# KAISTChangmin/MPMAvatar

Hardware: AMD Instinct MI355X
Metric: MPM substeps/sec (500k particles, 256^3 grid) (higher is better)
Workload: dtype f32; 1 GPU; sheet-500k; scene_name=sheet-497762, n_particles=497762, n_elements=331298, n_vertices=166464, n_traditional=0, n_grid=256, mode=fast, parallelism=single, n_active_nodes=148974, n_collider_nodes=32541, n_mover_nodes=0, n_active_blocks=10021, rebins=10, fallback_particles=0

## Files before the change

mpmavatar_amd/csrc/fast_device.hpp:

```cpp
#pragma once
#include <hip/hip_ext.h>
#include <algorithm>
#include <array>
#include <cstring>
#include <string.h>
#include <cstdlib>
#include <dlfcn.h>

#include <rccl/rccl.h>

#include <atomic>
#include <thread>

#include <rocprim/device/device_radix_sort.hpp>
#include <rocprim/device/device_scan.hpp>

#include "bc.hpp"
#include "ctx.hpp"
#include "mpm_math.hpp"

namespace mpm {
inline namespace fk {


// ... 36 lines not shown
__device__ __forceinline__ void st3(const Soa &a, int c0, int i, V3 v) {
  a.at(c0, i) = v.x; a.at(c0 + 1, i) = v.y; a.at(c0 + 2, i) = v.z;
}
__device__ __forceinline__ M3 ld9(const Soa &a, int c0, int i) {
  return M3{a.at(c0, i), a.at(c0 + 1, i), a.at(c0 + 2, i), a.at(c0 + 3, i), a.at(c0 + 4, i),
            a.at(c0 + 5, i), a.at(c0 + 6, i), a.at(c0 + 7, i), a.at(c0 + 8, i)};
}
__device__ __forceinline__ void st9(const Soa &a, int c0, int i, const M3 &m) {
  a.at(c0, i) = m.a00; a.at(c0 + 1, i) = m.a01; a.at(c0 + 2, i) = m.a02; a.at(c0 + 3, i) = m.a10;
  a.at(c0 + 4, i) = m.a11; a.at(c0 + 5, i) = m.a12; a.at(c0 + 6, i) = m.a20; a.at(c0 + 7, i) = m.a21;
  a.at(c0 + 8, i) = m.a22;
}

enum { A_X = 0, A_V = 3, A_C = 6, A_MASS = 15, A_NC = 16 };
enum { N_STRESS = 0, N_VOL = 9, N_MU = 10, N_LAM = 11, N_NC = 12 };
enum { E_D = 0, E_RINV = 9, E_GAMMA = 12, E_KAPPA = 13, E_NC = 14 };
enum { T_F = 0, T_FT = 9, T_YS = 18, T_NC = 19 };
enum { GCH_MV = 4, GCH_VOUT = 4, GCH_COL = 8, GCH_MOV = 4 };

struct Bufs {
  Soa all, nv, el, tr;
  int *face_orig;
  int *sel;
};

struct Dims {
  int n_p, n_e, n_nv, n_v, n_t;
  int G, NB;
  float dx, inv_dx, grid_lim;
};
// ... 100 lines not shown

enum { SIG_PROGRESS = 1, SIG_DFLAG = 2, SIG_DSEQ = 3, SIG_RING0 = 8, SIG_RING_N = 16, SIG_WORDS = 32 };
static_assert(SIG_RING0 + SIG_RING_N <= SIG_WORDS && (SIG_RING_N & (SIG_RING_N - 1)) == 0, "signal ring must fit its buffer");
enum {
  CNT_FALLBACK = 0, CNT_DROPPED = 1,
  CNT_NCOL = 2, CNT_NMOV = 3,
  CNT_ACTIVE = 4,
  CNT_FACE = 5, CNT_DRIFT = 6,
  CNT_DRIFT_ALL = 7,
  CNT_EXP0 = 8, CNT_EXP1 = 9,
  CNT_LINK_TIMEOUT = 10, CNT_LINK_BAD = 11,
  CNT_LINK_VOTE = 12, CNT_LINK_VOTE_ALL = 13,
  CNT_BODY_MOVES = 14,
  CNT_PAR0 = 16,
  CNT_MMIN = 24, CNT_MMAX = 25, CNT_NSEL = 26,
  CNT_N = 32
};
constexpr int CNT_STATS_N = 8;
static_assert(CNT_NCOL + 1 == CNT_NMOV && CNT_LINK_TIMEOUT + 1 == CNT_LINK_BAD && CNT_LINK_VOTE + 1 == CNT_LINK_VOTE_ALL &&
              CNT_MMIN + 1 == CNT_MMAX && CNT_MMAX + 1 == CNT_NSEL, "counter slots that are copied or cleared as one range");
static_assert(CNT_ACTIVE < CNT_STATS_N && CNT_BODY_MOVES < CNT_PAR0 && CNT_PAR0 + 4 <= CNT_MMIN && CNT_NSEL < CNT_N, "counter layout");

constexpr int PEER_TAB = 8;
struct HaloIn {
  const int *slot;
  const float *buf[PEER_TAB];
  const int *sig[PEER_TAB];
  int n_peers, seq, ch;
};

struct GridPtrs {
  float *mv;
  float *vout;
  float *col;
  float *mov;
// ... 100 lines not shown
    if (m != 0.0f || px != 0.0f || py != 0.0f || pz != 0.0f) { pm[0] = 0.0f; pm[64] = 0.0f; pm[128] = 0.0f; pm[192] = 0.0f; }
    if (l == 0) z.m_flag[blk] = 0;
  }
  if (z.has_col && z.col_flag[blk]) {
    float *pc = z.col + ((size_t)blk * GCH_COL) * 64 + l;
    if (pc[0] != 0.0f) { pc[0] = 0.0f; pc[64] = 0.0f; pc[128] = 0.0f; pc[192] = 0.0f; pc[256] = 0.0f; pc[320] = 0.0f; pc[384] = 0.0f; }
    if (l == 0) z.col_flag[blk] = 0;
  }
  if (z.has_mov) {
    float *pv = z.mov + ((size_t)blk * GCH_MOV) * 64 + l;
    if (pv[0] != 0.0f) { pv[0] = 0.0f; pv[64] = 0.0f; pv[128] = 0.0f; pv[192] = 0.0f; }
  }
}


template <bool FINALIZE>
__device__ __forceinline__ void stress_elem_body(int e, const Bufs &b, F3 *ef, const Dims &d, float friction_coeff, const int *face_slot,
                                                 const SortKey *skeys, int blk_bits, int *counters, int step_id) {
  if (e >= d.n_e) return;
  const int sel = b.sel[e];
  int s1 = 0, s2 = 0, s3 = 0;
  SortKey sk = 0;
  M3 dm;
  if (FINALIZE) {
    s1 = face_slot[e]; s2 = face_slot[d.n_e + e]; s3 = face_slot[2 * d.n_e + e];
    sk = skeys[e];
    dm = m3_zero();
    dm.a02 = b.el.at(E_D + 2, e); dm.a12 = b.el.at(E_D + 5, e); dm.a22 = b.el.at(E_D + 8, e);
  } else {
    dm = ld9(b.el, E_D, e);
  }
  float gamma = b.el.at(E_GAMMA, e), kappa = b.el.at(E_KAPPA, e);
  V3 rinv = ld3(b.el, E_RINV, e);
  float vol = b.nv.at(N_VOL, e), mu = b.nv.at(N_MU, e), lam = b.nv.at(N_LAM, e);
  asm volatile("" : "+v"(s1), "+v"(s2), "+v"(s3), "+v"(sk), "+v"(dm.a02), "+v"(dm.a12), "+v"(dm.a22));
  asm volatile("" : "+v"(gamma), "+v"(kappa), "+v"(rinv.x), "+v"(rinv.y), "+v"(rinv.z), "+v"(vol), "+v"(mu), "+v"(lam));
  if (sel == 1) {
    for (int c = 0; c < 3; ++c) ef[c * d.n_e + e] = F3{0.0f, 0.0f, 0.0f};
    return;
  }
  V3 xe = v3(0, 0, 0), ve = v3(0, 0, 0);
  if (FINALIZE) {
    int v1 = d.n_nv + s1, v2 = d.n_nv + s2, v3i = d.n_nv + s3;
    V3 x1 = ld3(b.all, A_X, v1), x2 = ld3(b.all, A_X, v2), x3 = ld3(b.all, A_X, v3i);
    V3 u1 = ld3(b.all, A_V, v1), u2 = ld3(b.all, A_V, v2), u3 = ld3(b.all, A_V, v3i);
    ve = v3((u1.x + u2.x + u3.x) / 3.0f, (u1.y + u2.y + u3.y) / 3.0f, (u1.z + u2.z + u3.z) / 3.0f);
    xe = v3((x1.x + x2.x + x3.x) / 3.0f, (x1.y + x2.y + x3.y) / 3.0f, (x1.z + x2.z + x3.z) / 3.0f);
    V3 d1 = x2 - x1, d2 = x3 - x1;
    dm = m3_cols(d1, d2, v3(dm.a02, dm.a12, dm.a22));
  }
  QR3 q = qr_cloth(dm);
  float r02, r12, r22;
  V3 d3 = anisotropy_return_mapping(q, gamma, kappa, friction_coeff, r02, r12, r22);
  M3 stress;
  V3 f1, f2, f3;
  kirchhoff_anisotropy(q, r02, r12, r22, d3, rinv, vol, mu, lam, gamma, kappa, stress, f1, f2, f3);
  if (FINALIZE) {
    st3(b.all, A_V, e, ve);
    st3(b.all, A_X, e, xe);
  }
  b.el.at(E_D + 2, e) = d3.x; b.el.at(E_D + 5, e) = d3.y; b.el.at(E_D + 8, e) = d3.z;
  st9(b.nv, N_STRESS, e, stress);
  ef[e] = F3{f1.x, f1.y, f1.z};
  ef[d.n_e + e] = F3{f2.x, f2.y, f2.z};
  ef[2 * d.n_e + e] = F3{f3.x, f3.y, f3.z};
  if (FINALIZE) {
    int blk = key_block(sk, blk_bits);
    int oz = 4 * (blk % d.NB) - 1, oy = 4 * ((blk / d.NB) % d.NB) - 1, ox = 4 * (blk / (d.NB * d.NB)) - 1;
    int nbx = (int)(xe.x * d.inv_dx - 0.5f) - ox, nby = (int)(xe.y * d.inv_dx - 0.5f) - oy, nbz = (int)(xe.z * d.inv_dx - 0.5f) - oz;
    if (sel == 0 && ((unsigned)nbx > 5u || (unsigned)nby > 5u || (unsigned)nbz > 5u)) raise_drift(counters, step_id);
  }
}


constexpr int TS_I = 99, TS_J = 9;
constexpr int TILE_PAD = 768;
__device__ __forceinline__ int tile_idx(int i, int j, int k) { return i * TS_I + j * TS_J + k; }
// ... 139 lines not shown
```

mpmavatar_amd/csrc/fast_state.hpp:

```cpp
#pragma once
#include "g2p_device.hpp"

namespace mpm {


struct DistPeer : mpmhip_dist_peer {
  DistPeer() : mpmhip_dist_peer{} {}
  explicit DistPeer(const mpmhip_dist_peer &p) : mpmhip_dist_peer(p) {}
  float *link_local = nullptr, *link_remote = nullptr;
  int link_cap = 0;
  int *link_cnt = nullptr;
};

struct Rccl {
  void *h = nullptr;
  ncclResult_t (*GetUniqueId)(ncclUniqueId *) = nullptr;
  ncclResult_t (*CommInitRank)(ncclComm_t *, int, ncclUniqueId, int) = nullptr;
  ncclResult_t (*CommDestroy)(ncclComm_t) = nullptr;
  ncclResult_t (*GroupStart)() = nullptr;
  ncclResult_t (*GroupEnd)() = nullptr;
  ncclResult_t (*Send)(const void *, size_t, ncclDataType_t, int, ncclComm_t, hipStream_t) = nullptr;
  ncclResult_t (*Recv)(void *, size_t, ncclDataType_t, int, ncclComm_t, hipStream_t) = nullptr;
  ncclResult_t (*AllGather)(const void *, void *, size_t, ncclDataType_t, ncclComm_t, hipStream_t) = nullptr;
  ncclResult_t (*AllReduce)(const void *, void *, size_t, ncclDataType_t, ncclRedOp_t, ncclComm_t, hipStream_t) = nullptr;
// ... 43 lines not shown
    q.ghost_send = ghost_send; q.ghost_recv = ghost_recv;
    q.link_local = link_local; q.link_remote = link_remote; q.link_cap = link_cap; q.link_cnt = link_cnt;
    return q;
  }
};

constexpr int HALO_CHANNELS_MAX = 8;
inline int halo_channels(bool movers) { return movers ? 8 : 4; }
constexpr size_t halo_floats(size_t n_blocks, int channels) { return n_blocks * (size_t)channels * 64; }
constexpr size_t ghost_floats(size_t n_p, size_t n_e) { return 6 * n_p + 3 * n_e; }
constexpr int LINK_DATA0 = 32, LINK_FLAG_STRIDE = 16;
constexpr size_t link_arena_floats(int cap) { return (size_t)LINK_DATA0 + 2 * halo_floats((size_t)cap, HALO_CHANNELS_MAX); }
inline float *link_data(float *arena, int par, int cap) { return arena + LINK_DATA0 + (size_t)par * halo_floats((size_t)cap, HALO_CHANNELS_MAX); }
inline int *link_flag(float *arena, int par) { return (int *)arena + par * LINK_FLAG_STRIDE; }

constexpr int PIN_SCAN_N = 2, PIN_STATS_N = CNT_STATS_N, PIN_RCNT_N = RC_N, PIN_MASS_N = 3;
enum {
  PIN_SCAN = 0,
  PIN_STATS = PIN_SCAN + PIN_SCAN_N,
  PIN_ADJ_K = PIN_STATS + PIN_STATS_N,
  PIN_DIST_DRIFT,
  PIN_LINK_VOTE,
  PIN_LINK_TIMEOUT,
  PIN_HALO_MULTI,
  PIN_BODY_MOVES,
  PIN_RCNT,
  PIN_MASS = PIN_RCNT + PIN_RCNT_N,
  PIN_N = PIN_MASS + PIN_MASS_N
};
static_assert(PIN_SCAN + PIN_SCAN_N <= PIN_STATS && PIN_STATS + PIN_STATS_N <= PIN_ADJ_K && PIN_ADJ_K < PIN_DIST_DRIFT &&
              PIN_BODY_MOVES < PIN_RCNT && PIN_RCNT + PIN_RCNT_N <= PIN_MASS && PIN_MASS + PIN_MASS_N <= PIN_N,
// ... 128 lines not shown
      return true;
    }
    bool resize(size_t want) { if (!reserve(want)) return false; n = want; return true; }
    bool push_back(const T &v) { if (n == cap && !reserve(n + 1)) return false; p[n++] = v; return true; }
    void clear() { n = 0; }
    size_t size() const { return n; }
    T *data() { return p; }
    T &operator[](size_t i) { return p[i]; }
    T *begin() { return p; }
    T *end() { return p + n; }
    void release() { if (p) (void)hipHostFree(p); p = nullptr; n = cap = 0; }
  };
  Pinned<int> h_ranges, h_plist;
  Pinned<ChunkRec> h_chunks, h_chunks_g;
  bool elem_pending = false;
  bool all_simulated = false;
  int steps_since_rebin = 0;
  volatile int *h_sig = nullptr;
  unsigned sig_seq = 0;
  unsigned sig_at_rebin = 0;
  bool face_flag_seen = false;
  int host_lead = 6;
  bool have_order = false;
  int64_t rebins = 0;
  int rebin_interval = 32;
  bool adaptive_rebin = true;
  bool fuse_grid = true, fuse_trad = true;
  AccumRing acc;
  int64_t n_col_kept = 0;
  bool col_keep = true;
// ... 61 lines not shown
```

mpmavatar_amd/csrc/g2p_device.hpp:

```cpp
#pragma once
#include "p2g_device.hpp"

namespace mpm {
inline namespace fk {

struct G2PResult {
  V3 v;
  M3 C, F;
};

__device__ __forceinline__ G2PResult g2p_finish(const Stencil &s, const Dims &d, V3 nv, V3 Mx, V3 My, V3 Mz, V3 Fx, V3 Fy,
                                                V3 Fz) {
  G2PResult r;
  r.v = nv;
  float c4 = 4.0f * d.inv_dx;
  r.C = m3_cols(c4 * (Mx - s.fx.x * nv), c4 * (My - s.fx.y * nv), c4 * (Mz - s.fx.z * nv));
  r.F = m3_cols(d.inv_dx * Fx, d.inv_dx * Fy, d.inv_dx * Fz);
  return r;
}

#ifndef G2P_D3_SWEEP
#define G2P_D3_SWEEP 1
#endif
template <bool B128>
// ... 201 lines not shown
  WGT(g, 1, 0);
  __builtin_amdgcn_s_setprio(3);
  int w = xcd_slice(wg, n_chunks);
  if (w < 0) return;
  const ChunkRec cm = recs[w];
  asm volatile("" ::"s"(cm.e0), "s"(cm.t0), "s"(cm.v0));
  int blk = cm.blk, chunk = cm.chunk;
  int bz = blk % d.NB, by = (blk / d.NB) % d.NB, bx = blk / (d.NB * d.NB);
  int ox = 4 * bx - 1, oy = 4 * by - 1, oz = 4 * bz - 1;
  int cls = 0, s = 0;
  bool valid = cm.map(chunk * CHUNK + (int)threadIdx.x, cls, s);
  V3 x, d3;
  {
    int sx_ = valid ? s : 0, se = (valid && cls == 0) ? s : 0;
    x = ld3(b.all, A_X, sx_);
    d3 = v3(b.el.at(E_D + 2, se), b.el.at(E_D + 5, se), b.el.at(E_D + 8, se));
  }
  constexpr int NPT = TILE3 / PT;
  int nbk[NPT], nlk[NPT], hsl[NPT];
  float am[NPT], apx[NPT], apy[NPT], apz[NPT];
#pragma unroll
  for (int u = 0; u < NPT; ++u) {
    int t = (int)threadIdx.x + u * PT;
    int ti = t >> 6, tj = (t >> 3) & 7, tk = t & 7;
    int gx = ox + ti, gy = oy + tj, gz = oz + tk;
    bool in = in_grid(gx, gy, gz, d.G);
    nbk[u] = in ? blk_of(gx, gy, gz, d.NB) : -1;
    nlk[u] = loc_of(gx, gy, gz);
    am[u] = apx[u] = apy[u] = apz[u] = 0.0f;
    if (FUSED && !MFLAG) {
      const float *pm = g.mv + ((size_t)(in ? nbk[u] : blk) * GCH_MV) * 64 + nlk[u];
// ... 273 lines not shown
```

mpmavatar_amd/csrc/mpm_math.hpp:

```cpp
#pragma once
#include <hip/hip_runtime.h>

namespace mpm {

struct V3 {
  float x, y, z;
};
struct M3 {
  float a00, a01, a02, a10, a11, a12, a20, a21, a22;
};

__host__ __device__ __forceinline__ V3 v3(float x, float y, float z) { return V3{x, y, z}; }
__device__ __forceinline__ V3 operator+(V3 a, V3 b) { return V3{a.x + b.x, a.y + b.y, a.z + b.z}; }
__device__ __forceinline__ V3 operator-(V3 a, V3 b) { return V3{a.x - b.x, a.y - b.y, a.z - b.z}; }
__device__ __forceinline__ V3 operator*(float s, V3 a) { return V3{s * a.x, s * a.y, s * a.z}; }
__device__ __forceinline__ V3 operator*(V3 a, float s) { return V3{s * a.x, s * a.y, s * a.z}; }
__device__ __forceinline__ float dot(V3 a, V3 b) { return a.x * b.x + a.y * b.y + a.z * b.z; }
__device__ __forceinline__ V3 cross(V3 a, V3 b) {
  return V3{a.y * b.z - a.z * b.y, a.z * b.x - a.x * b.z, a.x * b.y - a.y * b.x};
}
__device__ __forceinline__ float length(V3 a) { return sqrtf(dot(a, a)); }
__device__ __forceinline__ V3 normalize(V3 a) {
  float l = length(a);
  float inv = l > 0.0f ? 1.0f / l : 0.0f;
// ... 283 lines not shown
    r22 = 1.0f;
  } else {
    float fn = kappa * (1.0f - q.r22) * (1.0f - q.r22);
    float ff = gamma * sqrtf(q.r02 * q.r02 + q.r12 * q.r12);
    if (ff > friction_coeff * fn) {
      r02 = q.r02 * friction_coeff * fn / ff;
      r12 = q.r12 * friction_coeff * fn / ff;
    }
  }
  float ax = r02 * q.q0.x, ay = r02 * q.q0.y, az = r02 * q.q0.z;
  float bx = r12 * q.q1.x, by = r12 * q.q1.y, bz = r12 * q.q1.z;
  float cx = r22 * q.q2.x, cy = r22 * q.q2.y, cz = r22 * q.q2.z;
  return v3((ax + bx) + cx, (ay + by) + cy, (az + bz) + cz);
}

__device__ __forceinline__ void kirchhoff_anisotropy(const QR3 &q, float r02, float r12, float r22, V3 d3, V3 Rinv,
                                                     float vol, float mu, float lam, float gamma, float kappa,
                                                     M3 &stress, V3 &f1, V3 &f2, V3 &f3) {
  float iD11 = Rinv.x, iD12 = Rinv.y, iD22 = Rinv.z;
  float F11 = q.r00 * iD11;
  float F12 = q.r00 * iD12 + q.r01 * iD22;
  float F22 = q.r11 * iD22;
  float hx = F11 + F22, hy = -F12;
  float hn = sqrtf(hx * hx + hy * hy);
  float c = hx / hn, s = hy / hn;
  float J = F11 * F22;
  float lj = lam * (J - 1.0f), m2 = 2.0f * mu;
  float K00 = m2 * (F11 - c) + lj * F22;
  float K01 = m2 * (F12 + s);
  float K11 = m2 * (F22 - c) + lj * F11;
  float dr13 = gamma * r02, dr23 = gamma * r12;
  float dr33 = (r22 > 1.0f) ? 0.0f : -kappa * (1.0f - r22) * (1.0f - r22);
  float k00 = K00 * F11 + K01 * F12 + dr13 * r02;
  float k01 = K01 * F22 + dr13 * r12;
  float k02 = dr13 * r22;
  float k11 = K11 * F22 + dr23 * r12;
  float k12 = dr23 * r22;
  float k22 = dr33 * r22;
  M3 K3s = M3{k00, k01, k02, k01, k11, k12, k02, k12, k22};
  float invdet = 1.0f / (F11 * F22 * r22);
  M3 Rinvm = invdet * M3{F22 * r22, 0.0f, 0.0f, -F12 * r22, F11 * r22, 0.0f, F12 * r12 - r02 * F22, -F11 * r12, F11 * F22};
  M3 Q = m3_cols(q.q0, q.q1, q.q2);
  M3 P = Q * K3s * Rinvm;
  V3 P1 = col0(P), P2 = col1(P), P3 = col2(P);
  f2 = (-vol) * (iD11 * P1 + iD12 * P2);
  f3 = (-vol * iD22) * P2;
  f1 = -1.0f * (f2 + f3);
  stress = vol * outer(P3, d3);
}

struct Stencil {
  int bx, by, bz;
  V3 fx;
  V3 w0, w1, w2;
  V3 dw0, dw1, dw2;
};

__device__ __forceinline__ Stencil make_stencil(V3 x, float inv_dx) {
  Stencil s;
  V3 g = inv_dx * x;
  s.bx = (int)(g.x - 0.5f);
  s.by = (int)(g.y - 0.5f);
  s.bz = (int)(g.z - 0.5f);
// ... 40 lines not shown
```

mpmavatar_amd/csrc/p2g.hip:

```cpp
#include "fast_state.hpp"

namespace mpm {

namespace {

template <bool FINALIZE>
__global__ void k_stress_elem(Bufs b, F3 *ef, Dims d, float friction_coeff, const int *face_slot,
                              const SortKey *skeys, int blk_bits, int *counters, int step_id) {
  stress_elem_body<FINALIZE>(blockIdx.x * blockDim.x + threadIdx.x, b, ef, d, friction_coeff, face_slot, skeys, blk_bits, counters, step_id);
}


__global__ void k_stress_trad(Bufs b, Dims d, mpmhip_model_scalars sc, float dt) {
  int t = blockIdx.x * blockDim.x + threadIdx.x;
  if (t >= d.n_t) return;
  int s = t + d.n_e;
  if (b.sel[s] != 0) return;
  M3 Ft = ld9(b.tr, T_FT, t), F, stress;
  float mu = b.nv.at(N_MU, s), lam = b.nv.at(N_LAM, s), ys = b.tr.at(T_YS, t);
  int m = sc.material;
  TradParams tp{m, sc.alpha, sc.hardening, sc.xi, sc.plastic_viscosity, sc.softening};
  traditional_update(Ft, tp, mu, lam, ys, dt, F, stress);
  if (m == 1 || m == 5) b.tr.at(T_YS, t) = ys;
  if (m == 5) { b.nv.at(N_MU, s) = mu; b.nv.at(N_LAM, s) = lam; }
  st9(b.tr, T_F, t, F);
  st9(b.nv, N_STRESS, s, stress);
}

__global__ __launch_bounds__(TPB) void k_stress_elem_splat(Bufs b, F3 *ef, Dims d, float friction_coeff, const int *face_slot,
                                                           const SortKey *skeys, int blk_bits, int n_splat, GridPtrs g, SplatArgs sa) {
  __shared__ double tile[4 * TILE_PAD];
  if ((int)blockIdx.x < n_splat) {
    col_splat_wg<1>(tile, sa, (int)blockIdx.x, d, g);
    return;
  }
  stress_elem_body<true>(((int)blockIdx.x - n_splat) * (int)blockDim.x + (int)threadIdx.x, b, ef, d, friction_coeff, face_slot, skeys,
                         blk_bits, g.counters, g.step_id);
}


template <int STEPS, bool TRAD, bool JT, bool FX>
__global__ __launch_bounds__(PT) void k_p2g(const ChunkRec *recs, int n_chunks, Bufs b, VAdj va, Dims d, float rpic, float dt,
                                             GridPtrs g, SplatArgs sa, TradParams tp) {
  __shared__ double tile[P2G_TILE_DOUBLES];
  __shared__ int esc[CHUNK];
  __shared__ int esc_n;
  __shared__ float red[8];
  p2g_body<STEPS, TRAD, JT, FX>(recs, n_chunks, b, va, d, rpic, dt, g, sa, tp, tile, esc, esc_n, red, (int)blockIdx.x);
}
}

void launch_p2g(mpmhip_ctx *c, bool trad, bool jt, unsigned grid, int n_chunks, float dt, const SplatArgs &sa, const TradParams &tp) {
// ... 4 lines not shown
#define P2G_ARGS grid, PT, f->chunks, n_chunks, b, f->va(), d, rpic, dt, f->g, sa, tp
  if (!f->p2g_fixed_now) {
    if (trad && jt) kstamp_launch(c, k_p2g<3, true, true, false>, P2G_ARGS);
    else if (trad) kstamp_launch(c, k_p2g<3, true, false, false>, P2G_ARGS);
    else kstamp_launch(c, k_p2g<3, false, false, false>, P2G_ARGS);
  } else if (trad && jt) kstamp_launch(c, k_p2g<P2G_STEPS, true, true, true>, P2G_ARGS);
  else if (trad) kstamp_launch(c, k_p2g<P2G_STEPS, true, false, true>, P2G_ARGS);
  else kstamp_launch(c, k_p2g<P2G_STEPS, false, false, true>, P2G_ARGS);
#undef P2G_ARGS
}
void launch_stress_elem(mpmhip_ctx *c, int mode, const SplatArgs &sa) {
  FastState *f = c->fast;
  const Dims &d = f->d;
  const Bufs &b = f->buf[f->cur];
  hipStream_t s = c->stream;
  if (mode == 2)
    kstamp_launch(c, k_stress_elem_splat, nblk(d.n_e) + (unsigned)sa.n_fbins, TPB, b, f->eforce, d, c->sc.friction_coeff, f->face_slot,
                  f->keys[1], f->blk_bits, sa.n_fbins, f->g, sa);
  else if (mode == 1)
    kstamp_launch(c, k_stress_elem<true>, nblk(d.n_e), TPB, b, f->eforce, d, c->sc.friction_coeff, f->face_slot, f->keys[1], f->blk_bits,
                  f->g.counters, f->g.step_id);
  else
    hipLaunchKernelGGL(k_stress_elem<false>, nblk(d.n_e), TPB, 0, s, b, f->eforce, d, c->sc.friction_coeff, f->face_slot, f->keys[1],
                       f->blk_bits, f->g.counters, f->g.step_id);
}
void launch_stress_trad(mpmhip_ctx *c, float dt) {
  FastState *f = c->fast;
  hipLaunchKernelGGL(k_stress_trad, nblk(f->d.n_t), TPB, 0, c->stream, f->buf[f->cur], f->d, c->sc, dt);
}

}
```

mpmavatar_amd/csrc/p2g_device.hpp:

```cpp
#pragma once
#include "fast_device.hpp"

namespace mpm {
inline namespace fk {

__device__ __forceinline__ bool splat_ok(int G, const Stencil &s) {
  return s.bx >= 0 && s.bx < G - 3 && s.by >= 0 && s.by < G - 3 && s.bz >= 0 && s.bz < G - 3;
}


__device__ __forceinline__ V3 face_centroid(const float *pts, const float *vel, float adv, const int32_t *idx, int f,
                                            V3 &p0, V3 &p1, V3 &p2) {
  int i0 = idx[3 * f], i1 = idx[3 * f + 1], i2 = idx[3 * f + 2];
  p0 = mesh_point(pts, vel, adv, i0); p1 = mesh_point(pts, vel, adv, i1); p2 = mesh_point(pts, vel, adv, i2);
  return v3((p0.x + p1.x + p2.x) / 3.0f, (p0.y + p1.y + p2.y) / 3.0f, (p0.z + p1.z + p2.z) / 3.0f);
}

struct FaceBin { int blk, start, cnt, pad; };

struct JointSplatArgs {
  const float *vel_t, *vel_v, *vel_f;
  int n_t, n_v, n_f;
  int off_t, off_v;
  const int *inv;
// ... 103 lines not shown
  int r;
  asm("v_cvt_rpi_i32_f32 %0, %1" : "=v"(r) : "v"(x));
  return r;
}

constexpr float DRIFT_LOOKAHEAD = 10.0f, DRIFT_LOOKAHEAD_DIST = 20.0f;
struct P2GRaw {
  V3 x, v;
  float mass, vol;
  M3 C, S;
  float mu, lam, ys;
  AdjBatch ab;
};
template <bool TRAD>
__device__ __forceinline__ P2GRaw p2g_issue(const Bufs &b, const VAdj &va, bool valid, int cls, int s, const Dims &d,
                                            bool w_nv, bool w_v) {
  P2GRaw r;
  int sa = valid ? s : 0;
  r.x = ld3(b.all, A_X, sa);
  r.mass = b.all.at(A_MASS, sa);
  r.C = ld9(b.all, A_C, sa);
  r.v = ld3(b.all, A_V, sa);
  r.S = m3_zero();
  r.vol = 1.0f;
  r.mu = r.lam = r.ys = 0.0f;
  if (w_nv) {
    int sn = (valid && cls != 2) ? s : 0;
    if (TRAD) {
      bool tr = valid && cls == 1;
      int t = tr ? s - d.n_e : 0;
      const float *base = tr ? b.tr.p + (size_t)T_FT * b.tr.n + t : b.nv.p + (size_t)N_STRESS * b.nv.n + sn;
      size_t st = tr ? (size_t)b.tr.n : (size_t)b.nv.n;
      r.S = M3{base[0], base[st], base[2 * st], base[3 * st], base[4 * st], base[5 * st], base[6 * st], base[7 * st], base[8 * st]};
      r.mu = b.nv.at(N_MU, sn);
      r.lam = b.nv.at(N_LAM, sn);
      if (d.n_t) r.ys = b.tr.at(T_YS, t);
    } else {
      r.S = ld9(b.nv, N_STRESS, sn);
    }
    r.vol = b.nv.at(N_VOL, sn);
  }
#pragma unroll
  for (int u = 0; u < ADJ_BATCH; ++u) r.ab.ent[u] = -1;
  if (w_v) r.ab = adj_load(va, (valid && cls == 2) ? s - d.n_nv : 0, 0);
  return r;
}
template <bool TRAD>
__device__ __forceinline__ P2GParticle p2g_finish(const P2GRaw &r, const Bufs &b, const VAdj &va, bool valid, int cls, int s,
                                                  const Dims &d, float rpic, float dt, bool w_v, const TradParams &tp) {
  V3 vf = v3(0, 0, 0);
  if (w_v) {
    vf = adj_gather(va, r.ab, vf);
    int vl = (valid && cls == 2) ? s - d.n_nv : 0;
    for (int k0 = ADJ_BATCH; k0 < va.K; k0 += ADJ_BATCH) vf = adj_gather(va, adj_load(va, vl, k0), vf);
  }
  P2GParticle q;
  q.s = make_stencil(r.x, d.inv_dx);
  q.mass = r.mass;
  q.mass_s = r.mass;
  M3 C = r.C;
  C = (1.0f - rpic) * C + (rpic / 2.0f) * (C - transpose(C));
  if (rpic < -0.001f) C = m3_zero();
  q.a0 = r.v - d.dx * (C * q.s.fx);
  q.Cdx = d.dx * C;
  q.Sdt = m3_zero();
  q.vfdt = v3(0, 0, 0);
  if (valid && cls == 0) {
    q.Sdt = (-dt * d.inv_dx) * r.S;
  } else if (valid && cls == 1) {
    M3 S = r.S;
    if (TRAD) {
      int t = s - d.n_e;
      M3 F;
      float mu = r.mu, lam = r.lam, ys = r.ys;
      traditional_update(r.S, tp, mu, lam, ys, dt, F, S);
      if (tp.material == 1 || tp.material == 5) b.tr.at(T_YS, t) = ys;
      if (tp.material == 5) { b.nv.at(N_MU, s) = mu; b.nv.at(N_LAM, s) = lam; }
      st9(b.tr, T_F, t, F);
      st9(b.nv, N_STRESS, s, S);
    }
    q.Sdt = (-dt * d.inv_dx * r.vol) * S;
  } else if (valid) {
    q.vfdt = dt * vf;
  }
  return q;
}
template <bool TRAD>
__device__ __forceinline__ P2GParticle p2g_load(const Bufs &b, const VAdj &va, int cls, int s, const Dims &d, float rpic,
                                                float dt, const TradParams &tp) {
  P2GRaw r = p2g_issue<TRAD>(b, va, true, cls, s, d, cls != 2, cls == 2);
  return p2g_finish<TRAD>(r, b, va, true, cls, s, d, rpic, dt, cls == 2, tp);
}

__device__ __forceinline__ int dpp_shr_i(int v, int old, int n) {
  switch (n) {
    case 1: return __builtin_amdgcn_update_dpp(old, v, 0x111, 0xf, 0xf, false);
    case 2: return __builtin_amdgcn_update_dpp(old, v, 0x112, 0xf, 0xf, false);
    case 4: return __builtin_amdgcn_update_dpp(old, v, 0x114, 0xf, 0xf, false);
    default: return __builtin_amdgcn_update_dpp(old, v, 0x118, 0xf, 0xf, false);
  }
}
__device__ __forceinline__ float dpp_shr_f(float v, int n) { return __int_as_float(dpp_shr_i(__float_as_int(v), 0, n)); }

struct SegMask {
  float m1, m2, m4, m8;
// ... 535 lines not shown
    WGT(g, 0, 6);
    return;
  }
  int w = xcd_slice(bid - (sa.e0 == 0 ? sa.n_extra : 0), n_chunks);
  if (w < 0) { wg_done(sa.pack); return; }
  if (g.stagger > 0 && bid < g.stagger_first) {
    int slot = (int)(__builtin_amdgcn_s_getreg(63492) & 0xfu) % g.stagger_groups;
    for (int i = 0; i < slot * g.stagger; ++i) __builtin_amdgcn_s_sleep(16);
  }
  const ChunkRec cm = recs[w];
  int blk = cm.blk, chunk = cm.chunk;
  int bz = blk % d.NB, by = (blk / d.NB) % d.NB, bx = blk / (d.NB * d.NB);
  int ox = 4 * bx - 1, oy = 4 * by - 1, oz = 4 * bz - 1;
  int cls = 0, s = 0;
  bool valid = cm.map(chunk * CHUNK + (int)threadIdx.x, cls, s);
  bool w_nv = __any(valid && cls != 2), w_v = __any(valid && cls == 2);
  if (DBG(g, 8)) w_v = false;
  if (DBG(g, 16)) w_nv = false;
  WGT(g, 0, 1);
  P2GRaw raw = p2g_issue<TRAD>(b, va, valid, cls, s, d, w_nv, w_v);
  for (int t = threadIdx.x; t < ((FX && !JT) ? 2 : 4) * TILE_PAD; t += PT) tile[t] = 0.0;
  if (threadIdx.x == 0) esc_n = 0;
  if (valid) {
    float la = g.lookahead * dt;
    int fx = (int)((raw.x.x + la * raw.v.x) * d.inv_dx - 0.5f) - ox, fy = (int)((raw.x.y + la * raw.v.y) * d.inv_dx - 0.5f) - oy,
        fz = (int)((raw.x.z + la * raw.v.z) * d.inv_dx - 0.5f) - oz;
    if ((unsigned)fx > 5u || (unsigned)fy > 5u || (unsigned)fz > 5u) raise_drift(g.counters, g.step_id);
  }
  WGT(g, 0, 2);
  P2GParticle q = p2g_finish<TRAD>(raw, b, va, valid, cls, s, d, rpic, dt, w_v, tp);
  FxScale fs{1.0f, 1.0f, 1.0f, 1.0f};
  if (FX) {
    float bm, bp;
    fx_bounds(q, valid, bm, bp);
    fs = fx_scales(bm, bp, red);
// ... 55 lines not shown
```

mpmavatar_amd/csrc/resort.hip:

```cpp
#include "fast_state.hpp"

namespace mpm {

namespace {


__global__ void k_import(mpmhip_state_ptrs st, mpmhip_model_ptrs md, Bufs b, const int *perm, Dims d, int dist) {
  int s = blockIdx.x * blockDim.x + threadIdx.x;
  if (s >= d.n_p) return;
  int o = perm[s];
  for (int c = 0; c < 3; ++c) b.all.at(A_X + c, s) = st.particle_x[3 * (size_t)o + c];
  for (int c = 0; c < 3; ++c) b.all.at(A_V + c, s) = st.particle_v[3 * (size_t)o + c];
  for (int c = 0; c < 9; ++c) b.all.at(A_C + c, s) = st.particle_C[9 * (size_t)o + c];
  b.all.at(A_MASS, s) = st.particle_mass[o];
  int sel = st.particle_selection[o];
  b.sel[s] = dist ? sel : (sel != 0 ? 1 : 0);
  if (s < d.n_nv) {
    for (int c = 0; c < 9; ++c) b.nv.at(N_STRESS + c, s) = st.particle_stress[9 * (size_t)o + c];
    b.nv.at(N_VOL, s) = st.particle_vol[o];
    b.nv.at(N_MU, s) = md.mu[o];
    b.nv.at(N_LAM, s) = md.lam[o];
    if (s < d.n_e) {
      for (int c = 0; c < 9; ++c) b.el.at(E_D + c, s) = st.particle_d[9 * (size_t)o + c];
      for (int c = 0; c < 3; ++c) b.el.at(E_RINV + c, s) = st.particle_R_inv[3 * (size_t)o + c];
      b.el.at(E_GAMMA, s) = md.gamma[o];
      b.el.at(E_KAPPA, s) = md.kappa[o];
      for (int c = 0; c < 3; ++c) b.face_orig[c * d.n_e + s] = (int)st.faces[3 * (size_t)o + c];
    } else {
      int t = s - d.n_e;
      for (int c = 0; c < 9; ++c) b.tr.at(T_F + c, t) = st.particle_F[9 * (size_t)o + c];
      for (int c = 0; c < 9; ++c) b.tr.at(T_FT + c, t) = st.particle_F_trial[9 * (size_t)o + c];
      b.tr.at(T_YS, t) = md.yield_stress[o];
    }
  }
}


__global__ void k_export(mpmhip_state_ptrs st, mpmhip_model_ptrs md, Bufs b, VAdj va, const int *perm,
                         Dims d, int export_model) {
  int s = blockIdx.x * blockDim.x + threadIdx.x;
  if (s >= d.n_p) return;
  int o = perm[s];
  for (int c = 0; c < 3; ++c) st.particle_x[3 * (size_t)o + c] = b.all.at(A_X + c, s);
  for (int c = 0; c < 3; ++c) st.particle_v[3 * (size_t)o + c] = b.all.at(A_V + c, s);
  for (int c = 0; c < 9; ++c) st.particle_C[9 * (size_t)o + c] = b.all.at(A_C + c, s);
  if (s < d.n_nv) {
    for (int c = 0; c < 9; ++c) st.particle_stress[9 * (size_t)o + c] = b.nv.at(N_STRESS + c, s);
    if (s < d.n_e) {
      for (int c = 0; c < 9; ++c) st.particle_d[9 * (size_t)o + c] = b.el.at(E_D + c, s);
    } else {
      int t = s - d.n_e;
      for (int c = 0; c < 9; ++c) st.particle_F[9 * (size_t)o + c] = b.tr.at(T_F + c, t);
      for (int c = 0; c < 9; ++c) st.particle_F_trial[9 * (size_t)o + c] = b.tr.at(T_FT + c, t);
      if (export_model) {
        md.yield_stress[o] = b.tr.at(T_YS, t);
        md.mu[o] = b.nv.at(N_MU, s);
        md.lam[o] = b.nv.at(N_LAM, s);
      }
    }
  } else {
    int v = s - d.n_nv;
    store_v3(st.vertex_force + 3 * (size_t)(o - d.n_nv), vertex_force(va, v));
// ... 235 lines not shown
}


__global__ void k_mass_span(const float *mass, const int *sel, int n, int *counters) {
  int i = blockIdx.x * blockDim.x + threadIdx.x;
  float m = (i < n && sel[i] == 0) ? mass[i] : 0.0f;
  int lo = m > 0.0f ? __float_as_int(m) : 0x7f7fffff, hi = m > 0.0f ? __float_as_int(m) : 0;
#pragma unroll
  for (int o = 32; o > 0; o >>= 1) { lo = min(lo, __shfl_xor(lo, o)); hi = max(hi, __shfl_xor(hi, o)); }
  if ((threadIdx.x & 63) == 0) { atomicMin(counters + CNT_MMIN, lo); atomicMax(counters + CNT_MMAX, hi); }
  unsigned long long ns = __ballot(i < n && sel[i] != 0);
  if ((threadIdx.x & 63) == 0 && ns) atomicAdd(counters + CNT_NSEL, (int)__popcll(ns));
}


__global__ __launch_bounds__(RS_TPB) void k_keys(Bufs b, Dims d, int kf, float lead, int ghost_g2p, SortKey *keys, int *iota, int *clear,
                                                 int n_clear, int *hist, int *gsum, int n_tiles, ZeroArgs z) {
  __shared__ int h[RS_BINS];
  if ((int)blockIdx.x >= n_tiles) {
    zero_blocks_wg(z, (int)blockIdx.x - n_tiles);
    return;
  }
  const int t = threadIdx.x, lane = t & 63, base = (int)blockIdx.x * RS_TILE;
  for (int i = (int)blockIdx.x * RS_TPB + t; i < n_clear; i += n_tiles * RS_TPB) clear[i] = 0;
  h[t] = 0;
  __syncthreads();
#pragma unroll
  for (int j = 0; j < RS_IPT; ++j) {
    int s = base + j * RS_TPB + t;
    bool in = s < d.n_p;
// ... 194 lines not shown
  return MPMHIP_OK;
}

int do_import(mpmhip_ctx *c) {
  FastState *f = c->fast;
  const Dims &d = f->d;
  if (!f->have_order) {
    if (d.n_p) hipLaunchKernelGGL(k_iota, nblk(d.n_p), TPB, 0, c->stream, f->perm[f->cur], d.n_p);
    f->have_order = true;
  }
  flush_g2p(c);
  if (d.n_p) {
    hipLaunchKernelGGL(k_import, nblk(d.n_p), TPB, 0, c->stream, c->st, c->md, f->buf[f->cur], f->perm[f->cur], d,
                       f->dist ? 1 : 0);
    MPM_HIP_CHECK(c, hipMemsetD32Async((hipDeviceptr_t)(f->g.counters + CNT_MMIN), 0x7f7fffff, 1, c->stream));
    MPM_HIP_CHECK(c, hipMemsetD32Async((hipDeviceptr_t)(f->g.counters + CNT_MMAX), 0, 2, c->stream));
    hipLaunchKernelGGL(k_mass_span, nblk(d.n_p), TPB, 0, c->stream, (const float *)c->st.particle_mass, (const int *)c->st.particle_selection,
                       d.n_p, f->g.counters);
    f->mass_span_pending = true;
  }
  if (d.n_e && d.n_v) {
    hipStream_t s = c->stream;
    MPM_HIP_CHECK(c, hipMemsetAsync(f->adj_cnt, 0, ((size_t)d.n_v + 1) * sizeof(int), s));
    hipLaunchKernelGGL(k_adj_build, nblk(d.n_e), TPB, 0, s, c->st.faces, d.n_e, d.n_v, f->adj_cnt, (int *)nullptr, 0, 0);
    hipLaunchKernelGGL(k_max_int, nblk(d.n_v), TPB, 0, s, f->adj_cnt, d.n_v, f->adj_cnt + d.n_v);
    MPM_HIP_CHECK(c, hipMemcpyAsync(f->h_pin + PIN_ADJ_K, f->adj_cnt + d.n_v, sizeof(int), hipMemcpyDeviceToHost, s));
    MPM_HIP_CHECK(c, hipStreamSynchronize(s));
    int K = std::max(f->h_pin[PIN_ADJ_K], 1);
    if (K > f->adj_cap) {
      int rc2;
      if ((rc2 = dalloc(c, &f->adj_o, (size_t)K * d.n_v, false))) return rc2;
      if ((rc2 = dalloc(c, &f->adj_s, (size_t)K * d.n_v, false))) return rc2;
      f->adj_cap = K;
    }
    f->adj_K = K;
    MPM_HIP_CHECK(c, hipMemsetAsync(f->adj_o, 0xff, (size_t)K * d.n_v * sizeof(int), s));
    MPM_HIP_CHECK(c, hipMemsetAsync(f->adj_cnt, 0, (size_t)d.n_v * sizeof(int), s));
    hipLaunchKernelGGL(k_adj_build, nblk(d.n_e), TPB, 0, s, c->st.faces, d.n_e, d.n_v, f->adj_cnt, f->adj_o, K, 1);
    MPM_HIP_CHECK(c, hipMemsetAsync(f->eforce, 0, ((size_t)3 * d.n_e + 1) * sizeof(F3), s));
  }
  f->elem_pending = false;
  c->caller_dirty = false;
  c->internal_dirty = false;
  f->steps_since_rebin = 1 << 30;
  return MPMHIP_OK;
}

constexpr int RS_MAX_N = 1 << 21;
static bool sort_custom(const FastState *f, int n) { return !f->sort_rocprim && n <= RS_MAX_N; }
static int sort_passes(int bits) { return (bits + RS_BITS - 1) / RS_BITS; }
static int sort_input(const FastState *f, int n, int bits) { return sort_custom(f, n) ? 1 - (sort_passes(bits) & 1) : 0; }
static int sort_reserve(mpmhip_ctx *c, int n) {
  FastState *f = c->fast;
  const int tiles = (n + RS_TILE - 1) / RS_TILE, groups = (tiles + RS_GROUP - 1) / RS_GROUP;
  if (tiles > f->rs_tiles) {
    int rc;
// ... 122 lines not shown
                       cap_A, f->rcnt, (int)RC_NA, 2, (int *)nullptr, 0);
    hipLaunchKernelGGL(k_build_chunks, 1, 1024, 0, s, f->plist, f->ranges, cap_P, f->rcnt, f->chunks, f->chunks + cap_ch, cap_ch, f->g.counters);
    if (with_faces)
      hipLaunchKernelGGL(k_fbin_compact, nblk(cap_A), TPB, 0, s, f->alist, f->rcnt, cap_A, f->fb_start, f->fb_cnt, f->fbins, cap_fb);
    MPM_HIP_CHECK(c, hipMemcpyAsync(f->h_pin + PIN_RCNT, f->rcnt, PIN_RCNT_N * sizeof(int), hipMemcpyDeviceToHost, s));
    if (f->mass_span_pending)
      MPM_HIP_CHECK(c, hipMemcpyAsync(f->h_pin + PIN_MASS, f->g.counters + CNT_MMIN, PIN_MASS_N * sizeof(int), hipMemcpyDeviceToHost, s));
    MPM_HIP_CHECK(c, hipStreamSynchronize(s));
    if (f->mass_span_pending) {
      float lo, hi;
      const int *hm = f->h_pin + PIN_MASS;
      memcpy(&lo, hm, 4); memcpy(&hi, hm + (CNT_MMAX - CNT_MMIN), 4);
      f->mass_span = (hi > 0.0f && lo < 3.0e38f) ? hi / lo : 1.0f;
      f->p2g_fixed_now = f->p2g_fixed && (f->p2g_fixed_forced || std::max(f->mass_span, f->global_mass_span) <= 1.0e5f);
      f->all_simulated = hm[CNT_NSEL - CNT_MMIN] == 0;
      f->mass_span_pending = false;
    }
    const int *h = f->h_pin + PIN_RCNT;
    if (h[RC_OVER]) {
      f->cap_P = std::max(f->cap_P, std::min(nb, std::max(h[RC_NP], (h[RC_NCH] - d.n_p / CHUNK)) * 2 + 1024));
      if (h[RC_OVER] & ~1) f->cap_P = std::min(nb, f->cap_P * 2);
      continue;
    }
    f->n_P = h[RC_NP];
    f->n_A = h[RC_NA];
    f->acc.end_relist(relist, f->alist, f->n_A);
    f->n_chunks = h[RC_NCH];
    const bool any_ghost = h[RC_GHOST] != 0;
    f->n_chunks_g = any_ghost ? h[RC_NCHG] : f->n_chunks;
    f->chunks_g = any_ghost ? f->chunks + cap_ch : f->chunks;
// ... 15 lines not shown
  }
  f->sig_at_rebin = f->sig_seq;
  f->g.ab_flag = f->ab_flag;
  f->steps_since_rebin = 0;
  f->rebins += 1;
  return MPMHIP_OK;
}

int fast_pull(mpmhip_ctx *c) {
  FastState *f = c->fast;
  const Dims &d = f->d;
  flush_elements(c);
  if (d.n_p && f->have_order) {
    int m = c->sc.material;
    hipLaunchKernelGGL(k_export, nblk(d.n_p), TPB, 0, c->stream, c->st, c->md, f->buf[f->cur], f->va(),
                       f->perm[f->cur], d, (m == 1 || m == 5) ? 1 : 0);
  }
  c->internal_dirty = false;
  return MPMHIP_OK;
}
int fast_debug_sort(mpmhip_ctx *c, const uint32_t *keys_in, int n, int bits, uint32_t *keys_out, int32_t *order_out) {
  FastState *f = c->fast;
  if (n == 0) return MPMHIP_OK;
  unsigned *kb[2] = {nullptr, nullptr};
  int *vtmp = nullptr;
  auto done = [&](int rc) {
    for (void *p : {(void *)kb[0], (void *)kb[1], (void *)vtmp}) if (p) (void)hipFree(p);
    return rc;
  };
  MPM_HIP_CHECK(c, hipMalloc(&kb[0], (size_t)n * sizeof(unsigned)));
  if (hipMalloc(&kb[1], (size_t)n * sizeof(unsigned)) != hipSuccess || hipMalloc(&vtmp, (size_t)n * sizeof(int)) != hipSuccess)
// ... 14 lines not shown
```

Measured before the change: 16190 substeps/s.

## Store element stress as rank-one factors and hoist uniform material constants

```diff
diff --git a/mpmavatar_amd/csrc/fast_device.hpp b/mpmavatar_amd/csrc/fast_device.hpp
--- a/mpmavatar_amd/csrc/fast_device.hpp
+++ b/mpmavatar_amd/csrc/fast_device.hpp
@@ -74,6 +74,7 @@
 
 enum { A_X = 0, A_V = 3, A_C = 6, A_MASS = 15, A_NC = 16 };
 enum { N_STRESS = 0, N_VOL = 9, N_MU = 10, N_LAM = 11, N_NC = 12 };
+enum { N_P3 = N_STRESS, N_D3 = N_STRESS + 3 };
 enum { E_D = 0, E_RINV = 9, E_GAMMA = 12, E_KAPPA = 13, E_NC = 14 };
 enum { T_F = 0, T_FT = 9, T_YS = 18, T_NC = 19 };
 enum { GCH_MV = 4, GCH_VOUT = 4, GCH_COL = 8, GCH_MOV = 4 };
@@ -204,11 +205,13 @@
   CNT_BODY_MOVES = 14,
   CNT_PAR0 = 16,
   CNT_MMIN = 24, CNT_MMAX = 25, CNT_NSEL = 26,
+  CNT_EC_DIFF = 27, CNT_EC_VAL = 28,
   CNT_N = 32
 };
 constexpr int CNT_STATS_N = 8;
 static_assert(CNT_NCOL + 1 == CNT_NMOV && CNT_LINK_TIMEOUT + 1 == CNT_LINK_BAD && CNT_LINK_VOTE + 1 == CNT_LINK_VOTE_ALL &&
-              CNT_MMIN + 1 == CNT_MMAX && CNT_MMAX + 1 == CNT_NSEL, "counter slots that are copied or cleared as one range");
+              CNT_MMIN + 1 == CNT_MMAX && CNT_MMAX + 1 == CNT_NSEL && CNT_NSEL + 1 == CNT_EC_DIFF && CNT_EC_DIFF + 1 == CNT_EC_VAL &&
+              CNT_EC_VAL + 4 == CNT_N, "counter slots that are copied or cleared as one range");
 static_assert(CNT_ACTIVE < CNT_STATS_N && CNT_BODY_MOVES < CNT_PAR0 && CNT_PAR0 + 4 <= CNT_MMIN && CNT_NSEL < CNT_N, "counter layout");
 
 constexpr int PEER_TAB = 8;
@@ -339,9 +342,13 @@
 }
 
 
+struct ElemConsts {
+  float gamma, kappa, mu, lam;
+  int uniform;
+};
 template <bool FINALIZE>
 __device__ __forceinline__ void stress_elem_body(int e, const Bufs &b, F3 *ef, const Dims &d, float friction_coeff, const int *face_slot,
-                                                 const SortKey *skeys, int blk_bits, int *counters, int step_id) {
+                                                 const SortKey *skeys, int blk_bits, int *counters, int step_id, const ElemConsts &ec) {
   if (e >= d.n_e) return;
   const int sel = b.sel[e];
   int s1 = 0, s2 = 0, s3 = 0;
@@ -355,9 +362,13 @@
   } else {
     dm = ld9(b.el, E_D, e);
   }
-  float gamma = b.el.at(E_GAMMA, e), kappa = b.el.at(E_KAPPA, e);
   V3 rinv = ld3(b.el, E_RINV, e);
-  float vol = b.nv.at(N_VOL, e), mu = b.nv.at(N_MU, e), lam = b.nv.at(N_LAM, e);
+  float vol = b.nv.at(N_VOL, e);
+  float gamma = ec.gamma, kappa = ec.kappa, mu = ec.mu, lam = ec.lam;
+  if (!ec.uniform) {
+    gamma = b.el.at(E_GAMMA, e); kappa = b.el.at(E_KAPPA, e);
+    mu = b.nv.at(N_MU, e); lam = b.nv.at(N_LAM, e);
+  }
   asm volatile("" : "+v"(s1), "+v"(s2), "+v"(s3), "+v"(sk), "+v"(dm.a02), "+v"(dm.a12), "+v"(dm.a22));
   asm volatile("" : "+v"(gamma), "+v"(kappa), "+v"(rinv.x), "+v"(rinv.y), "+v"(rinv.z), "+v"(vol), "+v"(mu), "+v"(lam));
   if (sel == 1) {
@@ -377,15 +388,14 @@
   QR3 q = qr_cloth(dm);
   float r02, r12, r22;
   V3 d3 = anisotropy_return_mapping(q, gamma, kappa, friction_coeff, r02, r12, r22);
-  M3 stress;
   V3 f1, f2, f3;
-  kirchhoff_anisotropy(q, r02, r12, r22, d3, rinv, vol, mu, lam, gamma, kappa, stress, f1, f2, f3);
+  V3 P3 = kirchhoff_anisotropy_factor(q, r02, r12, r22, rinv, vol, mu, lam, gamma, kappa, f1, f2, f3);
   if (FINALIZE) {
     st3(b.all, A_V, e, ve);
     st3(b.all, A_X, e, xe);
   }
-  b.el.at(E_D + 2, e) = d3.x; b.el.at(E_D + 5, e) = d3.y; b.el.at(E_D + 8, e) = d3.z;
-  st9(b.nv, N_STRESS, e, stress);
+  st3(b.nv, N_P3, e, P3);
+  st3(b.nv, N_D3, e, d3);
   ef[e] = F3{f1.x, f1.y, f1.z};
   ef[d.n_e + e] = F3{f2.x, f2.y, f2.z};
   ef[2 * d.n_e + e] = F3{f3.x, f3.y, f3.z};
diff --git a/mpmavatar_amd/csrc/fast_state.hpp b/mpmavatar_amd/csrc/fast_state.hpp
--- a/mpmavatar_amd/csrc/fast_state.hpp
+++ b/mpmavatar_amd/csrc/fast_state.hpp
@@ -81,7 +81,7 @@
 inline float *link_data(float *arena, int par, int cap) { return arena + LINK_DATA0 + (size_t)par * halo_floats((size_t)cap, HALO_CHANNELS_MAX); }
 inline int *link_flag(float *arena, int par) { return (int *)arena + par * LINK_FLAG_STRIDE; }
 
-constexpr int PIN_SCAN_N = 2, PIN_STATS_N = CNT_STATS_N, PIN_RCNT_N = RC_N, PIN_MASS_N = 3;
+constexpr int PIN_SCAN_N = 2, PIN_STATS_N = CNT_STATS_N, PIN_RCNT_N = RC_N, PIN_MASS_N = CNT_N - CNT_MMIN;
 enum {
   PIN_SCAN = 0,
   PIN_STATS = PIN_SCAN + PIN_SCAN_N,
@@ -240,6 +240,8 @@
   Pinned<int> h_ranges, h_plist;
   Pinned<ChunkRec> h_chunks, h_chunks_g;
   bool elem_pending = false;
+  bool elem_stress_factored = false;
+  ElemConsts elem_consts{0.0f, 0.0f, 0.0f, 0.0f, 0};
   bool all_simulated = false;
   int steps_since_rebin = 0;
   volatile int *h_sig = nullptr;
diff --git a/mpmavatar_amd/csrc/g2p_device.hpp b/mpmavatar_amd/csrc/g2p_device.hpp
--- a/mpmavatar_amd/csrc/g2p_device.hpp
+++ b/mpmavatar_amd/csrc/g2p_device.hpp
@@ -239,7 +239,7 @@
   {
     int sx_ = valid ? s : 0, se = (valid && cls == 0) ? s : 0;
     x = ld3(b.all, A_X, sx_);
-    d3 = v3(b.el.at(E_D + 2, se), b.el.at(E_D + 5, se), b.el.at(E_D + 8, se));
+    d3 = ld3(b.nv, N_D3, se);
   }
   constexpr int NPT = TILE3 / PT;
   int nbk[NPT], nlk[NPT], hsl[NPT];
diff --git a/mpmavatar_amd/csrc/mpm_math.hpp b/mpmavatar_amd/csrc/mpm_math.hpp
--- a/mpmavatar_amd/csrc/mpm_math.hpp
+++ b/mpmavatar_amd/csrc/mpm_math.hpp
@@ -321,9 +321,11 @@
   return v3((ax + bx) + cx, (ay + by) + cy, (az + bz) + cz);
 }
 
-__device__ __forceinline__ void kirchhoff_anisotropy(const QR3 &q, float r02, float r12, float r22, V3 d3, V3 Rinv,
-                                                     float vol, float mu, float lam, float gamma, float kappa,
-                                                     M3 &stress, V3 &f1, V3 &f2, V3 &f3) {
+__device__ __forceinline__ M3 stress_from_factors(float vol, V3 P3, V3 d3) { return vol * outer(P3, d3); }
+
+__device__ __forceinline__ V3 kirchhoff_anisotropy_factor(const QR3 &q, float r02, float r12, float r22, V3 Rinv,
+                                                          float vol, float mu, float lam, float gamma, float kappa,
+                                                          V3 &f1, V3 &f2, V3 &f3) {
   float iD11 = Rinv.x, iD12 = Rinv.y, iD22 = Rinv.z;
   float F11 = q.r00 * iD11;
   float F12 = q.r00 * iD12 + q.r01 * iD22;
@@ -353,7 +355,13 @@
   f2 = (-vol) * (iD11 * P1 + iD12 * P2);
   f3 = (-vol * iD22) * P2;
   f1 = -1.0f * (f2 + f3);
-  stress = vol * outer(P3, d3);
+  return P3;
+}
+__device__ __forceinline__ void kirchhoff_anisotropy(const QR3 &q, float r02, float r12, float r22, V3 d3, V3 Rinv,
+                                                     float vol, float mu, float lam, float gamma, float kappa,
+                                                     M3 &stress, V3 &f1, V3 &f2, V3 &f3) {
+  V3 P3 = kirchhoff_anisotropy_factor(q, r02, r12, r22, Rinv, vol, mu, lam, gamma, kappa, f1, f2, f3);
+  stress = stress_from_factors(vol, P3, d3);
 }
 
 struct Stencil {
diff --git a/mpmavatar_amd/csrc/p2g.hip b/mpmavatar_amd/csrc/p2g.hip
--- a/mpmavatar_amd/csrc/p2g.hip
+++ b/mpmavatar_amd/csrc/p2g.hip
@@ -6,8 +6,8 @@
 
 template <bool FINALIZE>
 __global__ void k_stress_elem(Bufs b, F3 *ef, Dims d, float friction_coeff, const int *face_slot,
-                              const SortKey *skeys, int blk_bits, int *counters, int step_id) {
-  stress_elem_body<FINALIZE>(blockIdx.x * blockDim.x + threadIdx.x, b, ef, d, friction_coeff, face_slot, skeys, blk_bits, counters, step_id);
+                              const SortKey *skeys, int blk_bits, int *counters, int step_id, ElemConsts ec) {
+  stress_elem_body<FINALIZE>(blockIdx.x * blockDim.x + threadIdx.x, b, ef, d, friction_coeff, face_slot, skeys, blk_bits, counters, step_id, ec);
 }
 
 
@@ -28,14 +28,15 @@
 }
 
 __global__ __launch_bounds__(TPB) void k_stress_elem_splat(Bufs b, F3 *ef, Dims d, float friction_coeff, const int *face_slot,
-                                                           const SortKey *skeys, int blk_bits, int n_splat, GridPtrs g, SplatArgs sa) {
+                                                           const SortKey *skeys, int blk_bits, int n_splat, GridPtrs g, SplatArgs sa,
+                                                           ElemConsts ec) {
   __shared__ double tile[4 * TILE_PAD];
   if ((int)blockIdx.x < n_splat) {
     col_splat_wg<1>(tile, sa, (int)blockIdx.x, d, g);
     return;
   }
   stress_elem_body<true>(((int)blockIdx.x - n_splat) * (int)blockDim.x + (int)threadIdx.x, b, ef, d, friction_coeff, face_slot, skeys,
-                         blk_bits, g.counters, g.step_id);
+                         blk_bits, g.counters, g.step_id, ec);
 }
 
 
@@ -70,15 +71,17 @@
   const Dims &d = f->d;
   const Bufs &b = f->buf[f->cur];
   hipStream_t s = c->stream;
+  const ElemConsts &ec = f->elem_consts;
+  f->elem_stress_factored = true;
   if (mode == 2)
     kstamp_launch(c, k_stress_elem_splat, nblk(d.n_e) + (unsigned)sa.n_fbins, TPB, b, f->eforce, d, c->sc.friction_coeff, f->face_slot,
-                  f->keys[1], f->blk_bits, sa.n_fbins, f->g, sa);
+                  f->keys[1], f->blk_bits, sa.n_fbins, f->g, sa, ec);
   else if (mode == 1)
     kstamp_launch(c, k_stress_elem<true>, nblk(d.n_e), TPB, b, f->eforce, d, c->sc.friction_coeff, f->face_slot, f->keys[1], f->blk_bits,
-                  f->g.counters, f->g.step_id);
+                  f->g.counters, f->g.step_id, ec);
   else
     hipLaunchKernelGGL(k_stress_elem<false>, nblk(d.n_e), TPB, 0, s, b, f->eforce, d, c->sc.friction_coeff, f->face_slot, f->keys[1],
-                       f->blk_bits, f->g.counters, f->g.step_id);
+                       f->blk_bits, f->g.counters, f->g.step_id, ec);
 }
 void launch_stress_trad(mpmhip_ctx *c, float dt) {
   FastState *f = c->fast;
diff --git a/mpmavatar_amd/csrc/p2g_device.hpp b/mpmavatar_amd/csrc/p2g_device.hpp
--- a/mpmavatar_amd/csrc/p2g_device.hpp
+++ b/mpmavatar_amd/csrc/p2g_device.hpp
@@ -141,7 +141,7 @@
 };
 template <bool TRAD>
 __device__ __forceinline__ P2GRaw p2g_issue(const Bufs &b, const VAdj &va, bool valid, int cls, int s, const Dims &d,
-                                            bool w_nv, bool w_v) {
+                                            bool w_nv, bool w_v, bool w_t) {
   P2GRaw r;
   int sa = valid ? s : 0;
   r.x = ld3(b.all, A_X, sa);
@@ -158,12 +158,15 @@
       int t = tr ? s - d.n_e : 0;
       const float *base = tr ? b.tr.p + (size_t)T_FT * b.tr.n + t : b.nv.p + (size_t)N_STRESS * b.nv.n + sn;
       size_t st = tr ? (size_t)b.tr.n : (size_t)b.nv.n;
-      r.S = M3{base[0], base[st], base[2 * st], base[3 * st], base[4 * st], base[5 * st], base[6 * st], base[7 * st], base[8 * st]};
+      r.S = M3{base[0], base[st], base[2 * st], base[3 * st], base[4 * st], base[5 * st], 0.0f, 0.0f, 0.0f};
+      if (w_t) { r.S.a20 = base[6 * st]; r.S.a21 = base[7 * st]; r.S.a22 = base[8 * st]; }
       r.mu = b.nv.at(N_MU, sn);
       r.lam = b.nv.at(N_LAM, sn);
       if (d.n_t) r.ys = b.tr.at(T_YS, t);
     } else {
-      r.S = ld9(b.nv, N_STRESS, sn);
+      V3 s0 = ld3(b.nv, N_STRESS, sn), s1 = ld3(b.nv, N_STRESS + 3, sn), s2 = v3(0, 0, 0);
+      if (w_t) s2 = ld3(b.nv, N_STRESS + 6, sn);
+      r.S = M3{s0.x, s0.y, s0.z, s1.x, s1.y, s1.z, s2.x, s2.y, s2.z};
     }
     r.vol = b.nv.at(N_VOL, sn);
   }
@@ -193,7 +196,7 @@
   q.Sdt = m3_zero();
   q.vfdt = v3(0, 0, 0);
   if (valid && cls == 0) {
-    q.Sdt = (-dt * d.inv_dx) * r.S;
+    q.Sdt = (-dt * d.inv_dx) * stress_from_factors(r.vol, v3(r.S.a00, r.S.a01, r.S.a02), v3(r.S.a10, r.S.a11, r.S.a12));
   } else if (valid && cls == 1) {
     M3 S = r.S;
     if (TRAD) {
@@ -215,7 +218,7 @@
 template <bool TRAD>
 __device__ __forceinline__ P2GParticle p2g_load(const Bufs &b, const VAdj &va, int cls, int s, const Dims &d, float rpic,
                                                 float dt, const TradParams &tp) {
-  P2GRaw r = p2g_issue<TRAD>(b, va, true, cls, s, d, cls != 2, cls == 2);
+  P2GRaw r = p2g_issue<TRAD>(b, va, true, cls, s, d, cls != 2, cls == 2, cls == 1);
   return p2g_finish<TRAD>(r, b, va, true, cls, s, d, rpic, dt, cls == 2, tp);
 }
 
@@ -781,11 +784,11 @@
   int ox = 4 * bx - 1, oy = 4 * by - 1, oz = 4 * bz - 1;
   int cls = 0, s = 0;
   bool valid = cm.map(chunk * CHUNK + (int)threadIdx.x, cls, s);
-  bool w_nv = __any(valid && cls != 2), w_v = __any(valid && cls == 2);
+  bool w_nv = __any(valid && cls != 2), w_v = __any(valid && cls == 2), w_t = __any(valid && cls == 1);
   if (DBG(g, 8)) w_v = false;
   if (DBG(g, 16)) w_nv = false;
   WGT(g, 0, 1);
-  P2GRaw raw = p2g_issue<TRAD>(b, va, valid, cls, s, d, w_nv, w_v);
+  P2GRaw raw = p2g_issue<TRAD>(b, va, valid, cls, s, d, w_nv, w_v, w_t);
   for (int t = threadIdx.x; t < ((FX && !JT) ? 2 : 4) * TILE_PAD; t += PT) tile[t] = 0.0;
   if (threadIdx.x == 0) esc_n = 0;
   if (valid) {
diff --git a/mpmavatar_amd/csrc/resort.hip b/mpmavatar_amd/csrc/resort.hip
--- a/mpmavatar_amd/csrc/resort.hip
+++ b/mpmavatar_amd/csrc/resort.hip
@@ -37,7 +37,7 @@
 
 
 __global__ void k_export(mpmhip_state_ptrs st, mpmhip_model_ptrs md, Bufs b, VAdj va, const int *perm,
-                         Dims d, int export_model) {
+                         Dims d, int export_model, int factored) {
   int s = blockIdx.x * blockDim.x + threadIdx.x;
   if (s >= d.n_p) return;
   int o = perm[s];
@@ -45,7 +45,10 @@
   for (int c = 0; c < 3; ++c) st.particle_v[3 * (size_t)o + c] = b.all.at(A_V + c, s);
   for (int c = 0; c < 9; ++c) st.particle_C[9 * (size_t)o + c] = b.all.at(A_C + c, s);
   if (s < d.n_nv) {
-    for (int c = 0; c < 9; ++c) st.particle_stress[9 * (size_t)o + c] = b.nv.at(N_STRESS + c, s);
+    if (s < d.n_e && factored && b.sel[s] != 1)
+      store_m3(st.particle_stress + 9 * (size_t)o, stress_from_factors(b.nv.at(N_VOL, s), ld3(b.nv, N_P3, s), ld3(b.nv, N_D3, s)));
+    else
+      for (int c = 0; c < 9; ++c) st.particle_stress[9 * (size_t)o + c] = b.nv.at(N_STRESS + c, s);
     if (s < d.n_e) {
       for (int c = 0; c < 9; ++c) st.particle_d[9 * (size_t)o + c] = b.el.at(E_D + c, s);
     } else {
@@ -311,6 +314,20 @@
 }
 
 
+__global__ void k_elem_consts(const float *gamma, const float *kappa, const float *mu, const float *lam, int n_e, int *counters) {
+  int i = blockIdx.x * blockDim.x + threadIdx.x;
+  const unsigned *a[4] = {(const unsigned *)gamma, (const unsigned *)kappa, (const unsigned *)mu, (const unsigned *)lam};
+  bool differs = false;
+  if (i < n_e)
+    for (int k = 0; k < 4; ++k) {
+      unsigned v0 = a[k][0];
+      differs |= a[k][i] != v0;
+      if (i == 0) counters[CNT_EC_VAL + k] = (int)v0;
+    }
+  if (__ballot(differs) && (threadIdx.x & 63) == 0) counters[CNT_EC_DIFF] = 1;
+}
+
+
 __global__ __launch_bounds__(RS_TPB) void k_keys(Bufs b, Dims d, int kf, float lead, int ghost_g2p, SortKey *keys, int *iota, int *clear,
                                                  int n_clear, int *hist, int *gsum, int n_tiles, ZeroArgs z) {
   __shared__ int h[RS_BINS];
@@ -535,9 +552,13 @@
     hipLaunchKernelGGL(k_import, nblk(d.n_p), TPB, 0, c->stream, c->st, c->md, f->buf[f->cur], f->perm[f->cur], d,
                        f->dist ? 1 : 0);
     MPM_HIP_CHECK(c, hipMemsetD32Async((hipDeviceptr_t)(f->g.counters + CNT_MMIN), 0x7f7fffff, 1, c->stream));
-    MPM_HIP_CHECK(c, hipMemsetD32Async((hipDeviceptr_t)(f->g.counters + CNT_MMAX), 0, 2, c->stream));
+    MPM_HIP_CHECK(c, hipMemsetD32Async((hipDeviceptr_t)(f->g.counters + CNT_MMAX), 0, 3, c->stream));
     hipLaunchKernelGGL(k_mass_span, nblk(d.n_p), TPB, 0, c->stream, (const float *)c->st.particle_mass, (const int *)c->st.particle_selection,
                        d.n_p, f->g.counters);
+    if (d.n_e)
+      hipLaunchKernelGGL(k_elem_consts, nblk(d.n_e), TPB, 0, c->stream, (const float *)c->md.gamma, (const float *)c->md.kappa,
+                         (const float *)c->md.mu, (const float *)c->md.lam, d.n_e, f->g.counters);
+    f->elem_consts = ElemConsts{0.0f, 0.0f, 0.0f, 0.0f, 0};
     f->mass_span_pending = true;
   }
   if (d.n_e && d.n_v) {
@@ -561,6 +582,7 @@
     MPM_HIP_CHECK(c, hipMemsetAsync(f->eforce, 0, ((size_t)3 * d.n_e + 1) * sizeof(F3), s));
   }
   f->elem_pending = false;
+  f->elem_stress_factored = false;
   c->caller_dirty = false;
   c->internal_dirty = false;
   f->steps_since_rebin = 1 << 30;
@@ -713,6 +735,10 @@
       f->mass_span = (hi > 0.0f && lo < 3.0e38f) ? hi / lo : 1.0f;
       f->p2g_fixed_now = f->p2g_fixed && (f->p2g_fixed_forced || std::max(f->mass_span, f->global_mass_span) <= 1.0e5f);
       f->all_simulated = hm[CNT_NSEL - CNT_MMIN] == 0;
+      ElemConsts &ec = f->elem_consts;
+      ec.uniform = (d.n_e > 0 && hm[CNT_EC_DIFF - CNT_MMIN] == 0 && !getenv("MPMHIP_ELEM_CONSTS_PER_ELEMENT")) ? 1 : 0;
+      const int *hv = hm + (CNT_EC_VAL - CNT_MMIN);
+      memcpy(&ec.gamma, hv, 4); memcpy(&ec.kappa, hv + 1, 4); memcpy(&ec.mu, hv + 2, 4); memcpy(&ec.lam, hv + 3, 4);
       f->mass_span_pending = false;
     }
     const int *h = f->h_pin + PIN_RCNT;
@@ -758,7 +784,7 @@
   if (d.n_p && f->have_order) {
     int m = c->sc.material;
     hipLaunchKernelGGL(k_export, nblk(d.n_p), TPB, 0, c->stream, c->st, c->md, f->buf[f->cur], f->va(),
-                       f->perm[f->cur], d, (m == 1 || m == 5) ? 1 : 0);
+                       f->perm[f->cur], d, (m == 1 || m == 5) ? 1 : 0, f->elem_stress_factored ? 1 : 0);
   }
   c->internal_dirty = false;
   return MPMHIP_OK;
```

Result: no change. 16320 substeps/s (median of 6 runs) (+0.8%).
